# hku-mars/GS-SDF

Measured on NVIDIA H100. Metric: train_steps_per_s, higher is better.
Workload: dtype f32

## Files before the change

### gs-sdf_b200/csrc/sdf_grid.cuh

```cuda
#pragma once
#include <cuda_bf16.h>
#include <cuda_fp16.h>

#include "common.cuh"

namespace gssdf {

constexpr int kSdfThreads = 256;
constexpr int kMaxLevels = 16;
constexpr int kFeat = 32;

struct GridGeom {
    int L;
    uint32_t offset[kMaxLevels + 1];
    float scale[kMaxLevels];
    uint32_t res[kMaxLevels];
};

static inline float h_grid_scale(uint32_t level, float log2_pls, uint32_t base) { return exp2f(level * log2_pls) * base - 1.0f; }

static GridGeom make_grid(const gssdf_sdf_net &net) {
    GridGeom g;
    g.L = net.n_levels;
    uint32_t off = 0;
// ... 49 lines not shown
        p.pg[d] = (uint32_t)(int)t;
        p.pos[d] = v - t;
    }
    return p;
}

template <bool BRANCH_FREE = false>
__device__ __forceinline__ float2 encode_level(const __half2 *__restrict__ table, const GridGeom &g, int lvl, const float x[3]) {
    const __half2 *t = table + g.offset[lvl];
    const uint32_t hs = g.offset[lvl + 1] - g.offset[lvl];
    const LevelPos p = level_pos(x, g.scale[lvl]);
    __half2 vals[8];
    float w[8];
#pragma unroll
    for (int idx = 0; idx < 8; ++idx) {
        float wt = 1.f;
        uint32_t c[3];
#pragma unroll
        for (int d = 0; d < 3; ++d) {
            if ((idx & (1 << d)) == 0) { wt *= 1.f - p.pos[d]; c[d] = p.pg[d]; }
            else { wt *= p.pos[d]; c[d] = p.pg[d] + 1; }
        }
        w[idx] = wt;
        vals[idx] = __ldg(t + (BRANCH_FREE ? grid_index_sel : grid_index)(hs, g.res[lvl], c[0], c[1], c[2]));
    }
    __half2 r = __floats2half2_rn(0.f, 0.f);
#pragma unroll
    for (int idx = 0; idx < 8; ++idx) r = __hfma2(__float2half2_rn(w[idx]), vals[idx], r);
    return __half22float2(r);
}

struct Corners {
    uint32_t idx[8];
    float2 val[8];
};
__device__ __forceinline__ void load_corners(const __half2 *__restrict__ t, uint32_t hs, uint32_t res, const LevelPos &p, bool want_val, Corners &c) {
#pragma unroll
    for (int k = 0; k < 8; ++k)
        c.idx[k] = grid_index(hs, res, p.pg[0] + (k & 1), p.pg[1] + ((k >> 1) & 1), p.pg[2] + ((k >> 2) & 1));
    if (want_val) {
#pragma unroll
        for (int k = 0; k < 8; ++k) c.val[k] = __half22float2(__ldg(t + c.idx[k]));
    }
}
__device__ __forceinline__ int pair_left(int gd, int idx, const LevelPos &p, float &wt) {
    int cl = 0;
#pragma unroll
    for (int nd = 0; nd < 2; ++nd) {
        const int d = nd >= gd ? nd + 1 : nd;
        if ((idx & (1 << nd)) == 0) wt *= 1.f - p.pos[d];
        else { wt *= p.pos[d]; cl |= 1 << d; }
    }
    return cl;
}

__device__ __forceinline__ void encode_level_bwd(const __half2 *__restrict__ table, float *__restrict__ table_grad, const GridGeom &g,
                                                 int lvl, const float x[3], float g0, float g1, bool want_dx, float dx[3]) {
    const uint32_t hs = g.offset[lvl + 1] - g.offset[lvl];
    const LevelPos p = level_pos(x, g.scale[lvl]);
    const __half2 gh = __hmul2(__floats2half2_rn(g0, g1), __float2half2_rn(128.f));
    Corners c;
    load_corners(table + g.offset[lvl], hs, g.res[lvl], p, want_dx, c);
    if (table_grad) {
        float *tg = table_grad + 2 * (size_t)g.offset[lvl];
#pragma unroll
        for (int idx = 0; idx < 8; ++idx) {
            float wt = 1.f;
#pragma unroll
            for (int d = 0; d < 3; ++d) wt *= (idx & (1 << d)) == 0 ? 1.f - p.pos[d] : p.pos[d];
            const float2 v = __half22float2(__hmul2(__float2half2_rn(wt), gh));
            if (v.x != 0.f || v.y != 0.f)
                atomicAdd(reinterpret_cast<float2 *>(tg + 2 * (size_t)c.idx[idx]), make_float2(v.x * (1.f / 128.f), v.y * (1.f / 128.f)));
        }
    }
    if (want_dx) {
        const float2 ghf = __half22float2(gh);
#pragma unroll
        for (int gd = 0; gd < 3; ++gd) {
            float acc0 = 0.f, acc1 = 0.f;
#pragma unroll
            for (int idx = 0; idx < 4; ++idx) {
                float wt = g.scale[lvl];
                const int cl = pair_left(gd, idx, p, wt), cr = cl | (1 << gd);
                acc0 += wt * (c.val[cr].x - c.val[cl].x);
                acc1 += wt * (c.val[cr].y - c.val[cl].y);
            }
            dx[gd] = (ghf.x * acc0 + ghf.y * acc1) * (1.f / 128.f);
        }
    }
}

__device__ __forceinline__ void encode_level_bwd2(const __half2 *__restrict__ table, float *__restrict__ table_grad, const GridGeom &g,
                                                  int lvl, const float x[3], float dfeat0, float dfeat1, const float cc[3], float r[2]) {
    const uint32_t hs = g.offset[lvl + 1] - g.offset[lvl];
    const LevelPos p = level_pos(x, g.scale[lvl]);
    const __half2 gh = __hmul2(__floats2half2_rn(dfeat0, dfeat1), __float2half2_rn(128.f));
    Corners c;
    load_corners(table + g.offset[lvl], hs, g.res[lvl], p, true, c);
    float2 tacc[8];
#pragma unroll
    for (int k = 0; k < 8; ++k) tacc[k] = make_float2(0.f, 0.f);
    float r0 = 0.f, r1 = 0.f;
#pragma unroll
    for (int gd = 0; gd < 3; ++gd) {
        float acc0 = 0.f, acc1 = 0.f;
        const float grad_in = g.scale[lvl] * cc[gd];
#pragma unroll
        for (int idx = 0; idx < 4; ++idx) {
            float wd = g.scale[lvl], w = grad_in;
            const int cl = pair_left(gd, idx, p, wd);
            (void)pair_left(gd, idx, p, w);
            const int cr = cl | (1 << gd);
            acc0 += wd * (c.val[cr].x - c.val[cl].x);
            acc1 += wd * (c.val[cr].y - c.val[cl].y);
            if (table_grad) {
                const float2 vl = __half22float2(__hmul2(__float2half2_rn(-w), gh)), vr = __half22float2(__hmul2(__float2half2_rn(w), gh));
                tacc[cl].x += vl.x; tacc[cl].y += vl.y;
                tacc[cr].x += vr.x; tacc[cr].y += vr.y;
            }
        }
        r0 += acc0 * cc[gd];
        r1 += acc1 * cc[gd];
    }
    if (table_grad) {
        float *tg = table_grad + 2 * (size_t)g.offset[lvl];
#pragma unroll
        for (int k = 0; k < 8; ++k)
            if (tacc[k].x != 0.f || tacc[k].y != 0.f)
                atomicAdd(reinterpret_cast<float2 *>(tg + 2 * (size_t)c.idx[k]), make_float2(tacc[k].x * (1.f / 128.f), tacc[k].y * (1.f / 128.f)));
    }
    r[0] = __half2float(__float2half_rn(r0));
    r[1] = __half2float(__float2half_rn(r1));
}

__device__ __forceinline__ void load_x(const gssdf_sdf_net &net, const float *__restrict__ x, int64_t gi, int64_t n, float delta,
                                       float out[3]) {
    const int64_t i = gi % n;
    const int var = (int)(gi / n);
#pragma unroll
    for (int d = 0; d < 3; ++d) {
        float v = __ldg(x + 3 * i + d);
        if (var > 0 && (var - 1) / 2 == d) v += ((var - 1) & 1) ? -delta : delta;
        out[d] = net.inv_size != 0.f ? __fadd_rn(__fmul_rn(__fsub_rn(v, net.origin[d]), net.inv_size), 0.5f) : v;
    }
}


}
```

### gs-sdf_b200/csrc/sdf_tc.cu

```cuda
#include "sdf_grid.cuh"
#include "sdf_loss.cuh"

namespace gssdf {

constexpr int kFwdTcThreads = 512;
constexpr int kBwdTcThreads = 512;
constexpr int kLevels = 16;
static_assert(128 * kLevels == 4 * kBwdTcThreads, "encode batches assume 4 tasks per thread");
constexpr uint32_t kWImg = 24576;
constexpr uint32_t kGW = 3072;
constexpr uint32_t kGA = 2048;
constexpr uint32_t kGA0 = 1024;
constexpr uint32_t kGL = 1024;

__device__ __forceinline__ uint32_t off_act(int r, int k, int part) {
    return (uint32_t)((r >> 3) * kGA + part * 1024 + (k >> 3) * 128 + (r & 7) * 16 + (k & 7) * 2);
}
__device__ __forceinline__ uint32_t off_feat(int r, int k, int part) {
    return (uint32_t)((r >> 3) * kGA0 + part * 512 + (k >> 3) * 128 + (r & 7) * 16 + (k & 7) * 2);
}
__device__ __forceinline__ uint32_t off_lo(int r, int k) { return (uint32_t)((r >> 3) * kGL + (k >> 3) * 128 + (r & 7) * 16 + (k & 7) * 2); }
__device__ __host__ __forceinline__ uint32_t off_w(int o, int k, int part) {
    return (uint32_t)((o >> 3) * kGW + part * 1024 + (k >> 3) * 128 + (o & 7) * 16 + (k & 7) * 2);
}
// ... 295 lines not shown
                float act[32];
#pragma unroll
                for (int e = 0; e < 32; ++e) act[e] = fmaxf(d[e] + s_bias[l * 64 + 8 * (e >> 2) + fc + (e & 1)], 0.f);
                if (l < nh - 1) {
#pragma unroll
                    for (int e = 0; e < 32; e += 2) store2(sA, sL, fr + 8 * ((e >> 1) & 1), 8 * (e >> 2) + fc, act[e], act[e + 1]);
                } else {
                    float p0[2] = {0.f, 0.f}, p1[2] = {0.f, 0.f};
#pragma unroll
                    for (int e = 0; e < 32; ++e) {
                        const int i = (e >> 1) & 1, c = 8 * (e >> 2) + fc + (e & 1);
                        p0[i] = fmaf(act[e], s_wout[c], p0[i]);
                        p1[i] = fmaf(act[e], s_wout[HID + c], p1[i]);
                    }
#pragma unroll
                    for (int i = 0; i < 2; ++i) {
                        const float s0 = quad_sum(p0[i]), s1 = quad_sum(p1[i]);
                        const int p = fr + 8 * i;
                        bool live;
                        const int64_t e = eval_of(tile, p, live);
                        if ((lane & 3) == 0 && live) {
                            a.sdf[e] = s0 + s_wout[2 * HID];
                            if (a.y1) a.y1[e] = s1 + s_wout[2 * HID + 1];
                        }
                    }
                }
            }
            ++k;
        }
    }
    if (!ok) __trap();
}

constexpr size_t kBwdTcMain = 16 * kGA0 + 3 * 16 * kGA + 16 * kGA + 16 * kGL + kWImg;
constexpr size_t kBwdTcMisc = sizeof(float) * (4 * 64 + 132 + 384 + 4 * 128);
constexpr size_t kBwdTcMiscAnalytic = 128 * 16 * sizeof(uint16_t) + 128 * 3 * sizeof(float) + 64;
constexpr size_t bwd_tc_smem(bool analytic) { return kBwdTcMain + kBwdTcMisc + (analytic ? kBwdTcMiscAnalytic : 0); }
static_assert(bwd_tc_smem(true) + 1024 + 128 <= 196 * 1024, "the analytic variant must fit the 196 KiB shared-memory carve-out");

struct TcLossArgs {
    const float *gt_sdf, *weights, *visibilities;
    SdfLossCfg cfg;
    float *loss_out;
    int analytic;
    float align_weight;
    const float *sdf_variants;
    const uint8_t *valid_mask;
    const int32_t *n_gate;
};

template <bool FUSED, bool ANALYTIC>
__global__ void __launch_bounds__(kBwdTcThreads, 1)
sdf_bwd_tc_kernel(const gssdf_sdf_bwd_args a, const TcLossArgs lo, const GridGeom g, int64_t n_tiles) {
    constexpr int TM = 128, HID = 64, NT = kBwdTcThreads;
    extern __shared__ __align__(128) unsigned char s_tc[];
    unsigned char *sF = s_tc;
    unsigned char *sAct = sF + 16 * kGA0;
    unsigned char *sG = sAct + 3 * 16 * kGA;
    unsigned char *sL = sG + 16 * kGA;
    unsigned char *sW = sL + 16 * kGL;
    float *s_bias = reinterpret_cast<float *>(sW + kWImg);
    float *s_wout = s_bias + 4 * 64;
    float *s_dx = s_wout + 132;
    float *s_seed = s_dx;
    float *s_col = s_dx + 384;
    uint16_t *s_mask16 = reinterpret_cast<uint16_t *>(s_col + 4 * 128);
    float *s_gnum = s_col + 4 * 128 + 1024;
    int64_t *s_tbase = reinterpret_cast<int64_t *>(s_gnum + 384);
    __shared__ __align__(8) uint64_t s_wbar;

    const int tid = threadIdx.x, warp = tid >> 5, lane = tid & 31;
    const int q = warp & 3, cq = warp >> 2, row = 32 * q + lane, col0 = 16 * cq;
    const int wg = warp >> 2, fr = 16 * (warp & 3) + (lane >> 2), fc = 2 * (lane & 3);
    const int dr = 64 * (wg & 1) + fr, dc = 32 * (wg >> 1) + fc;
    const int nh = 1 + a.net.n_hidden;
    const int64_t n_eval = a.n * max(a.n_variants, 1);
    const int64_t n_live = a.n_live ? min((int64_t)*a.n_live, a.n) : a.n;
    const __half2 *table = reinterpret_cast<const __half2 *>(a.net.table_half);
    const unsigned char *wimg = reinterpret_cast<const unsigned char *>(a.net.mlp_packed);
    const int V = max(a.n_variants, 1), PT = FUSED ? TM / V : TM;
    float loss_acc = 0.f;
    constexpr bool analytic = ANALYTIC;
    static_assert(FUSED || !ANALYTIC, "the analytic eikonal path is part of the fused train kernel");
    float acc2_wo = 0.f;
    int n_coll = 0;

    if (tid == 0) {
        mbar_init(&s_wbar, 1);
        fence_mbar_init();
    }
    {
        const float *W = a.net.mlp;
        for (int l = 0; l < nh; ++l) {
            const int K = l == 0 ? kFeat : HID;
            if (tid < HID) s_bias[l * 64 + tid] = __ldg(W + (size_t)HID * K + tid);
            W += (size_t)HID * K + HID;
        }
        for (int e = tid; e < 2 * HID + 2; e += NT) s_wout[e] = __ldg(W + e);
    }
    __syncthreads();
    uint32_t ph_w = 0;
    bool ok = true, first_tile = true;
    float dbias[4] = {0.f, 0.f, 0.f, 0.f};
    float dwo0 = 0.f, dwo1 = 0.f, dbo = 0.f;
    float accW[32];
#pragma unroll
    for (int e = 0; e < 32; ++e) accW[e] = 0.f;
    float dD[16];

    auto sync_w = [&](bool wait) {
        fence_proxy_async();
        bool landed = true;
        if (wait) { landed = mbar_wait_bounded(&s_wbar, ph_w); ph_w ^= 1; }
        ok = __syncthreads_and(landed) && ok;
    };
    auto load_w = [&](int l) {
        mbar_arrive_expect_tx(&s_wbar, kWImg);
        bulk_g2s(sW, wimg + (size_t)l * kWImg, kWImg, &s_wbar);
    };
    auto finish = [&]() {
        wg_wait();
        acc_fence(dD);
        __syncthreads();
    };
    auto issue_gw = [&]() {
        const uint32_t gB = smem_u32(sG) + 8 * (wg & 1) * kGA, wB = smem_u32(sW) + 4 * (wg >> 1) * 128;
        wg_fence();
#pragma unroll
        for (int ks = 0; ks < HID / 16; ++ks) {
            const uint64_t gh = make_desc(gB + ks * 256, 128, kGA), gm = make_desc(gB + 1024 + ks * 256, 128, kGA);
            const uint64_t wh = make_desc(wB + ks * 2 * kGW, kGW, 128), wm = make_desc(wB + 1024 + ks * 2 * kGW, kGW, 128);
            wgmma_bf16<0, 1>(dD, gh, wh, ks > 0 ? 1u : 0u);
            wgmma_bf16<0, 1>(dD, gh, wm, 1);
            wgmma_bf16<0, 1>(dD, gm, wh, 1);
            wgmma_bf16<0, 1>(dD, gm, wm, 1);
        }
        wg_commit();
    };
    auto issue_dw = [&](int l) {
        if (wg != l) return;
        const uint32_t aB = smem_u32(l == 0 ? sF : sAct + (l - 1) * 16 * kGA), ga = l == 0 ? kGA0 : kGA, am = l == 0 ? 512u : 1024u;
        const uint32_t gB = smem_u32(sG);
        wg_fence();
#pragma unroll
        for (int ks = 0; ks < TM / 16; ++ks) {
            const uint64_t ah = make_desc(aB + ks * 2 * ga, ga, 128), amd = make_desc(aB + am + ks * 2 * ga, ga, 128);
            const uint64_t gh = make_desc(gB + ks * 2 * kGA, kGA, 128), gm = make_desc(gB + 1024 + ks * 2 * kGA, kGA, 128);
            wgmma_bf16<1, 1>(accW, ah, gh, 1);
            wgmma_bf16<1, 1>(accW, ah, gm, 1);
            wgmma_bf16<1, 1>(accW, amd, gh, 1);
            wgmma_bf16<1, 1>(accW, amd, gm, 1);
        }
        wg_commit();
    };


    auto second_order = [&]() {
        const int nc = n_coll;
        float *gf = reinterpret_cast<float *>(sL);
        float *s_cc = s_col;
        const float isz = a.net.inv_size != 0.f ? a.net.inv_size : 1.f;
        __syncthreads();
        for (int e = tid; e < (TM - nc) * 16; e += NT) s_mask16[nc * 16 + e] = 0;
        for (int e = tid; e < TM * 3; e += NT) s_dx[e] = 0.f;
        __syncthreads();
        auto seed_u = [&]() {
            const uint32_t bits = s_mask16[(row * 4 + nh - 1) * 4 + cq];
            float u[16];
#pragma unroll
            for (int j = 0; j < 16; ++j) u[j] = ((bits >> j) & 1u) ? s_wout[col0 + j] : 0.f;
            store8(sG, nullptr, row, col0, u);
            store8(sG, nullptr, row, col0 + 8, u + 8);
        };
        auto mask_bit = [&](int slot, int l, int e) -> bool {
            const int j = e >> 2;
            return (s_mask16[(slot * 4 + l - 1) * 4 + 2 * (wg >> 1) + (j >> 1)] >> (8 * (j & 1) + fc + (e & 1))) & 1u;
        };
        auto mask_store = [&](int l, unsigned char *dst) {
#pragma unroll
            for (int e = 0; e < 16; e += 2) {
                const int r = dr + 8 * ((e >> 1) & 1);
                store2(dst, nullptr, r, dc + 8 * (e >> 2), mask_bit(r, l, e) ? dD[e] : 0.f, mask_bit(r, l, e + 1) ? dD[e + 1] : 0.f);
            }
        };
        auto store_gf = [&]() {
            if (wg >> 1) return;
#pragma unroll
            for (int e = 0; e < 16; ++e) gf[(dr + 8 * ((e >> 1) & 1)) * 33 + dc + 8 * (e >> 2) + (e & 1)] = dD[e];
        };
        seed_u();
        if (tid == 0) { fence_proxy_async(); load_w(nh - 1); }
        for (int l = nh - 1; l >= 0 && ok; --l) {
            sync_w(true);
            if (!ok) return;
            issue_gw();
            finish();
            if (tid == 0 && l > 0) load_w(l - 1);
            if (l > 0) mask_store(l, sG);
            else store_gf();
        }
        __syncthreads();
        {
            static_assert(NT % TM == 0, "thread -> point mapping of the analytic pass");
            const int c = tid % TM;
            if (c < nc) {
                float x[3], acc[3] = {0.f, 0.f, 0.f};
                load_x(a.net, a.x, s_tbase[c / PT] + c % PT, a.n, a.delta, x);
#pragma unroll 1
                for (int lvl = tid / TM; lvl < kLevels; lvl += NT / TM) {
                    float dx[3] = {0.f, 0.f, 0.f};
                    encode_level_bwd(table, nullptr, g, lvl, x, gf[c * 33 + 2 * lvl], gf[c * 33 + 2 * lvl + 1], true, dx);
                    acc[0] += dx[0]; acc[1] += dx[1]; acc[2] += dx[2];
                }
                atomicAdd(&s_dx[c * 3 + 0], acc[0]);
                atomicAdd(&s_dx[c * 3 + 1], acc[1]);
                atomicAdd(&s_dx[c * 3 + 2], acc[2]);
            }
        }
        __syncthreads();
        if (tid < TM) {
            float cc[3] = {0.f, 0.f, 0.f};
            const SdfGate gate = tid < nc ? sdf_gate(lo.n_gate, lo.valid_mask, lo.visibilities, lo.cfg.visible_thr, s_tbase[tid / PT] + tid % PT)
                                          : SdfGate{false, true, 1.f};
            if (tid < nc && (!gate.gated || gate.gate)) {
                const float gx = s_dx[tid * 3] * isz, gy = s_dx[tid * 3 + 1] * isz, gz = s_dx[tid * 3 + 2] * isz;
                const float nl = gate.gated ? gate.ng : (float)n_live;
                const float nrm = sqrtf(gx * gx + gy * gy + gz * gz);
                const float we = lo.cfg.eikonal_weight / nl;
                loss_acc += we * (nrm - 1.f) * (nrm - 1.f);
                const float ke = nrm > 0.f ? 2.f * (nrm - 1.f) / nrm * we : 0.f;
                cc[0] = ke * gx; cc[1] = ke * gy; cc[2] = ke * gz;
                if (lo.align_weight > 0.f && (V == 7 || lo.sdf_variants)) {
                    const float wa = lo.align_weight / (3.f * nl);
                    const float *gn = s_gnum + tid * 3;
                    const float d0 = gx - gn[0], d1 = gy - gn[1], d2 = gz - gn[2];
                    loss_acc += wa * (fabsf(d0) + fabsf(d1) + fabsf(d2));
                    cc[0] += d0 > 0.f ? wa : (d0 < 0.f ? -wa : 0.f);
                    cc[1] += d1 > 0.f ? wa : (d1 < 0.f ? -wa : 0.f);
                    cc[2] += d2 > 0.f ? wa : (d2 < 0.f ? -wa : 0.f);
                }
            }
            s_cc[tid * 3] = cc[0] * isz; s_cc[tid * 3 + 1] = cc[1] * isz; s_cc[tid * 3 + 2] = cc[2] * isz;
        }
        __syncthreads();
#pragma unroll 1
        for (int task = tid; task < TM * kLevels; task += NT) {
            const int c = task % TM, lvl = task / TM;
            float r[2] = {0.f, 0.f};
            if (c < nc) {
                float x[3];
                load_x(a.net, a.x, s_tbase[c / PT] + c % PT, a.n, a.delta, x);
                encode_level_bwd2(table, a.table_grad, g, lvl, x, gf[c * 33 + 2 * lvl], gf[c * 33 + 2 * lvl + 1], s_cc + c * 3, r);
            }
            __nv_bfloat16 h0, m0, h1, m1;
            split2(r[0], h0, m0);
            split2(r[1], h1, m1);
            *reinterpret_cast<__nv_bfloat162 *>(sF + off_feat(c, 2 * lvl, 0)) = __halves2bfloat162(h0, h1);
            *reinterpret_cast<__nv_bfloat162 *>(sF + off_feat(c, 2 * lvl, 1)) = __halves2bfloat162(m0, m1);
        }
        if (!a.mlp_grad) { __syncthreads(); return; }
        __syncthreads();
        if (tid == 0) { fence_proxy_async(); load_w(0); }
        for (int l = 0; l < nh; ++l) {
            sync_w(true);
            if (!ok) return;
            issue_forward_layer<false>(dD, l, smem_u32(l == 0 ? sF + 8 * (wg & 1) * kGA0 : sAct + (l - 1) * 16 * kGA + 8 * (wg & 1) * kGA),
                                       0u, smem_u32(sW) + 4 * (wg >> 1) * kGW);
            finish();
            if (tid == 0 && (l + 1 < nh || nh > 1)) load_w(l + 1 < nh ? l + 1 : nh - 1);
            if (l < nh - 1) {
                mask_store(l + 1, sAct + l * 16 * kGA);
            } else {
#pragma unroll
                for (int e = 0; e < 16; e += 4) {
#pragma unroll
                    for (int c = 0; c < 2; ++c) {
                        float s = (mask_bit(dr, nh, e + c) ? dD[e + c] : 0.f) + (mask_bit(dr + 8, nh, e + 2 + c) ? dD[e + 2 + c] : 0.f);
                        s += __shfl_xor_sync(0xffffffffu, s, 4);
                        s += __shfl_xor_sync(0xffffffffu, s, 8);
                        s += __shfl_xor_sync(0xffffffffu, s, 16);
                        if (lane < 4) s_col[(4 * (wg & 1) + (warp & 3)) * 64 + dc + 2 * e + c] = s;
                    }
                }
            }
        }
        __syncthreads();
        if (q == 0 && lane < 16) {
            const int c = col0 + lane;
#pragma unroll
            for (int rg = 0; rg < 8; ++rg) acc2_wo += s_col[rg * 64 + c];
        }
        seed_u();
        for (int l = nh - 1; l >= 0 && ok; --l) {
            sync_w(l > 0);
            if (!ok) return;
            issue_dw(l);
            if (l > 0) issue_gw();
            finish();
            if (tid == 0 && l > 1) load_w(l - 1);
            if (l > 0) mask_store(l, sG);
        }
        __syncthreads();
    };

    for (int64_t tile = blockIdx.x; tile < n_tiles && ok; tile += gridDim.x) {
        const int64_t base = FUSED ? tile * PT : tile * TM;
        const int tm = (int)min((int64_t)TM, n_eval - base);
        if (FUSED ? base >= n_live : (base % a.n >= n_live && base % a.n + TM <= a.n)) continue;
        auto row_gi = [&](int p) -> int64_t {
            if (!FUSED) return min(base + p, n_eval - 1);
            const int j = p / V, v = p - j * V;
            return (int64_t)v * a.n + min(base + j, a.n - 1);
        };
        auto row_live = [&](int p) -> bool {
            if (!FUSED) return p < tm && (base + p) % a.n < n_live;
            const int j = p / V;
            return j < PT && base + j < n_live;
        };
        auto row_is_base = [&](int p) -> bool { return FUSED ? (p % V) == 0 : base + p < a.n; };
#define LIVE_TC(p_) row_live(p_)
        __syncthreads();
        if (tid == 0) {
            fence_proxy_async();
            load_w(0);
        }
        {
            float2 f[4];
#pragma unroll
            for (int i = 0; i < 4; ++i) {
                const int task = i * NT + tid, p = task % TM, lvl = task / TM;
                float x[3];
                load_x(a.net, a.x, row_gi(p), a.n, a.delta, x);
                f[i] = encode_level(table, g, lvl, x);
            }
#pragma unroll
            for (int i = 0; i < 4; ++i) {
                const int task = i * NT + tid, p = task % TM, lvl = task / TM;
                if (!LIVE_TC(p)) f[i] = make_float2(0.f, 0.f);
                __nv_bfloat16 h0, m0, h1, m1;
                split2(f[i].x, h0, m0);
                split2(f[i].y, h1, m1);
                *reinterpret_cast<__nv_bfloat162 *>(sF + off_feat(p, 2 * lvl, 0)) = __halves2bfloat162(h0, h1);
                *reinterpret_cast<__nv_bfloat162 *>(sF + off_feat(p, 2 * lvl, 1)) = __halves2bfloat162(m0, m1);
            }
        }
        if (!FUSED && tid < TM) {
            const bool lv = LIVE_TC(tid);
            s_seed[2 * tid] = lv ? __ldg(a.v_sdf + base + tid) : 0.f;
            s_seed[2 * tid + 1] = (lv && a.v_y1) ? __ldg(a.v_y1 + base + tid) : 0.f;
        }
        for (int l = 0; l < nh; ++l) {
            sync_w(true);
            if (!ok) break;
            issue_forward_layer(dD, l, smem_u32(l == 0 ? sF + 8 * (wg & 1) * kGA0 : sAct + (l - 1) * 16 * kGA + 8 * (wg & 1) * kGA),
                                smem_u32(sL + 8 * (wg & 1) * kGL), smem_u32(sW) + 4 * (wg >> 1) * kGW);
            finish();
            if (tid == 0 && l + 1 < nh) load_w(l + 1);
            float act[16];
#pragma unroll
            for (int e = 0; e < 16; ++e) act[e] = fmaxf(dD[e] + s_bias[l * 64 + dc + 8 * (e >> 2) + (e & 1)], 0.f);
            unsigned char *dst = (l < nh - 1) ? sAct + l * 16 * kGA : sG;
#pragma unroll
            for (int e = 0; e < 16; e += 2) store2(dst, l < nh - 1 ? sL : nullptr, dr + 8 * ((e >> 1) & 1), dc + 8 * (e >> 2), act[e], act[e + 1]);
            if (analytic) {
#pragma unroll
                for (int i = 0; i < 2; ++i) {
                    uint32_t bits[2] = {0u, 0u};
#pragma unroll
                    for (int j = 0; j < 4; ++j)
#pragma unroll
                        for (int c = 0; c < 2; ++c) bits[j >> 1] |= (act[4 * j + 2 * i + c] > 0.f ? 1u : 0u) << (8 * (j & 1) + fc + c);
#pragma unroll
                    for (int h = 0; h < 2; ++h) {
                        bits[h] |= __shfl_xor_sync(0xffffffffu, bits[h], 1);
                        bits[h] |= __shfl_xor_sync(0xffffffffu, bits[h], 2);
                    }
                    const int r = dr + 8 * i, jb = r / V;
                    if ((lane & 3) == 0 && r - jb * V == 0 && jb < PT && base + jb < n_live) {
                        s_mask16[((n_coll + jb) * 4 + l) * 4 + 2 * (wg >> 1)] = (uint16_t)bits[0];
                        s_mask16[((n_coll + jb) * 4 + l) * 4 + 2 * (wg >> 1) + 1] = (uint16_t)bits[1];
                    }
                }
            }
            if (FUSED && l == nh - 1) {
                float p0[2] = {0.f, 0.f}, p1[2] = {0.f, 0.f};
#pragma unroll
                for (int e = 0; e < 16; ++e) {
                    const int i = (e >> 1) & 1, c = dc + 8 * (e >> 2) + (e & 1);
                    p0[i] = fmaf(act[e], s_wout[c], p0[i]);
                    p1[i] = fmaf(act[e], s_wout[HID + c], p1[i]);
                }
                float *s_part = reinterpret_cast<float *>(sL);
#pragma unroll
                for (int i = 0; i < 2; ++i) {
                    const float s0 = quad_sum(p0[i]), s1 = quad_sum(p1[i]);
                    if ((lane & 3) == 0) {
                        s_part[((wg >> 1) * TM + dr + 8 * i) * 2] = s0;
                        s_part[((wg >> 1) * TM + dr + 8 * i) * 2 + 1] = s1;
                    }
                }
            }
        }
        if (!ok) break;
        __syncthreads();
        if (FUSED) {
            float *s_part = reinterpret_cast<float *>(sL), *s_out = s_part + 2 * TM * 2;
            if (tid < TM) {
                s_out[2 * tid] = s_part[tid * 2] + s_part[(TM + tid) * 2] + s_wout[2 * HID];
                s_out[2 * tid + 1] = s_part[tid * 2 + 1] + s_part[(TM + tid) * 2 + 1] + s_wout[2 * HID + 1];
                s_seed[2 * tid] = 0.f;
                s_seed[2 * tid + 1] = 0.f;
            }
            __syncthreads();
            if (tid < PT && base + tid < n_live) {
                const int64_t i = base + tid;
                float sv[7], v_s[7], v_y;
                for (int v = 0; v < V; ++v) sv[v] = s_out[2 * (tid * V + v)];
                SdfLossCfg cfg1 = lo.cfg;
                if (analytic) {
                    cfg1.eikonal_weight = 0.f;
                    if (tid == 0) s_tbase[n_coll / PT] = base;
                    if (V == 1 && lo.sdf_variants) {
                        for (int v = 1; v < 7; ++v) sv[v] = __ldg(lo.sdf_variants + (int64_t)v * a.n + i);
                    }
                    if (V == 7 || lo.sdf_variants) {
                        const float inv2d = 0.5f / lo.cfg.delta;
                        s_gnum[(n_coll + tid) * 3 + 0] = (sv[1] - sv[2]) * inv2d;
                        s_gnum[(n_coll + tid) * 3 + 1] = (sv[3] - sv[4]) * inv2d;
                        s_gnum[(n_coll + tid) * 3 + 2] = (sv[5] - sv[6]) * inv2d;
                    }
                }
                loss_acc += sdf_point_loss(cfg1, (float)n_live, V, sv, s_out[2 * tid * V + 1], lo.gt_sdf != nullptr,
                                           lo.gt_sdf ? __ldg(lo.gt_sdf + i) : 0.f, lo.weights != nullptr, lo.weights ? __ldg(lo.weights + i) : 0.f,
                                           lo.visibilities != nullptr, lo.visibilities ? __ldg(lo.visibilities + i) : 0.f, v_s, v_y,
                                           sdf_gate(lo.n_gate, lo.valid_mask, lo.visibilities, lo.cfg.visible_thr, i));
                for (int v = 0; v < V; ++v) s_seed[2 * (tid * V + v)] = v_s[v];
                s_seed[2 * tid * V + 1] = v_y;
            }
            __syncthreads();
        }
        {
            float an[16], gl[16];
            load8_sum(sG, row, col0, an);
            load8_sum(sG, row, col0 + 8, an + 8);
            const float v0 = s_seed[2 * row], v1 = s_seed[2 * row + 1];
#pragma unroll
            for (int j = 0; j < 16; ++j) gl[j] = an[j] > 0.f ? v0 * s_wout[col0 + j] + v1 * s_wout[HID + col0 + j] : 0.f;
            store8(sG, nullptr, row, col0, gl);
            store8(sG, nullptr, row, col0 + 8, gl + 8);
            if (a.mlp_grad) {
                float c0[16], c1[16];
#pragma unroll
                for (int j = 0; j < 16; ++j) { c0[j] = v0 * an[j]; c1[j] = v1 * an[j]; }
                const float s0 = colsum16(c0, lane), s1 = colsum16(c1, lane);
                if (lane < 16) {
                    s_col[q * 128 + col0 + lane] = s0;
                    s_col[q * 128 + 64 + col0 + lane] = s1;
                }
                if (cq == 0) {
                    const float b0 = warp_sum(v0), b1 = warp_sum(v1);
                    if (lane == 0) { s_dx[256 + 2 * q] = b0; s_dx[256 + 2 * q + 1] = b1; }
                }
            }
        }
        __syncthreads();
        if (a.mlp_grad) {
            if (tid < 2 * HID) {
                const float s = s_col[tid] + s_col[128 + tid] + s_col[256 + tid] + s_col[384 + tid];
                if (tid < HID) dwo0 += s; else dwo1 += s;
            } else if (tid < 2 * HID + 2) {
                const int o = tid - 2 * HID;
                dbo += s_dx[256 + o] + s_dx[258 + o] + s_dx[260 + o] + s_dx[262 + o];
            }
        }
        for (int l = nh - 1; l >= 0; --l) {
            sync_w(l < nh - 1);
            if (!ok) break;
            if (a.mlp_grad) issue_dw(l);
            issue_gw();
            if (a.mlp_grad) {
                float c[16];
                load8_sum(sG, row, col0, c);
                load8_sum(sG, row, col0 + 8, c + 8);
                const float s = colsum16(c, lane);
                if (lane < 16) s_col[q * 128 + col0 + lane] = s;
            }
            finish();
            if (tid == 0 && l > 0) load_w(l - 1);
            if (l > 0) {
#pragma unroll
                for (int e = 0; e < 16; e += 2) {
                    const int r = dr + 8 * ((e >> 1) & 1), c = dc + 8 * (e >> 2);
                    const float2 m = load2_hi(sAct + (l - 1) * 16 * kGA, r, c);
                    store2(sG, nullptr, r, c, m.x > 0.f ? dD[e] : 0.f, m.y > 0.f ? dD[e + 1] : 0.f);
                }
            } else if ((wg >> 1) == 0) {
                float *gf = reinterpret_cast<float *>(sL);
#pragma unroll
                for (int e = 0; e < 16; ++e) gf[(dr + 8 * ((e >> 1) & 1)) * 33 + dc + 8 * (e >> 2) + (e & 1)] = dD[e];
            }
            __syncthreads();
            if (a.mlp_grad && q == 0 && lane < 16) {
                const int c = col0 + lane;
                dbias[l] += s_col[c] + s_col[128 + c] + s_col[256 + c] + s_col[384 + c];
            }
        }
        if (!ok) break;
        for (int e = tid; e < TM * 3; e += NT) s_dx[e] = 0.f;
        __syncthreads();
        {
            const float *gf = reinterpret_cast<const float *>(sL);
            for (int task = tid; task < TM * g.L; task += NT) {
                const int p = task % TM, lvl = task / TM;
                if (LIVE_TC(p)) {
                    float x[3], dx[3] = {0.f, 0.f, 0.f};
                    load_x(a.net, a.x, row_gi(p), a.n, a.delta, x);
                    const bool want_dx = a.v_x != nullptr && row_is_base(p);
                    encode_level_bwd(table, a.table_grad, g, lvl, x, gf[p * 33 + 2 * lvl], gf[p * 33 + 2 * lvl + 1], want_dx, dx);
                    if (want_dx) {
                        atomicAdd(&s_dx[p * 3 + 0], dx[0]);
                        atomicAdd(&s_dx[p * 3 + 1], dx[1]);
                        atomicAdd(&s_dx[p * 3 + 2], dx[2]);
                    }
                }
            }
        }
        __syncthreads();
        if (a.v_x) {
            const float sc = a.net.inv_size != 0.f ? a.net.inv_size : 1.f;
            if (FUSED) {
                for (int e = tid; e < PT * 3; e += NT) {
                    const int j = e / 3, d = e - 3 * j;
                    if (base + j < n_live) a.v_x[(base + j) * 3 + d] = s_dx[(j * V) * 3 + d] * sc;
                }
            } else {
                for (int e = tid; e < tm * 3; e += NT)
                    if (base + e / 3 < n_live) a.v_x[base * 3 + e] = s_dx[e] * sc;
            }
        }
        first_tile = false;
        if (ANALYTIC) {
            n_coll += (int)min((int64_t)PT, n_live - base);
            if (n_coll + PT > TM) {
                second_order();
                n_coll = 0;
                if (!ok) break;
            }
        }

#undef LIVE_TC
    }
    if (ANALYTIC && ok && n_coll > 0) second_order();
    __syncthreads();
    if (ok && a.mlp_grad && !first_tile) {
        float *G = a.mlp_grad;
        for (int l = 0; l < nh; ++l) {
            const int K = l == 0 ? kFeat : HID;
            if (wg == l) {
#pragma unroll
                for (int e = 0; e < 32; ++e) {
                    const int k = fr + 8 * ((e >> 1) & 1), o = 8 * (e >> 2) + fc + (e & 1);
                    if (k < K) atomicAdd(G + (size_t)o * K + k, accW[e]);
                }
            }
            if (q == 0 && lane < 16) atomicAdd(G + (size_t)HID * K + col0 + lane, dbias[l]);
            G += (size_t)HID * K + HID;
        }
        if (ANALYTIC && q == 0 && lane < 16) atomicAdd(G + col0 + lane, acc2_wo);
        if (tid < HID) atomicAdd(G + tid, dwo0);
        else if (tid < 2 * HID) atomicAdd(G + tid, dwo1);
        else if (tid < 2 * HID + 2) atomicAdd(G + tid, dbo);
    }
    if (FUSED && lo.loss_out) {
        loss_acc = warp_sum(loss_acc);
        if (lane == 0 && loss_acc != 0.f) atomicAdd(lo.loss_out, loss_acc);
    }
    if (!ok) __trap();
}

}

using namespace gssdf;

extern "C" int64_t gssdf_sdf_mlp_packed_bytes(const gssdf_sdf_net *net) {
    if (!net || net->hidden_dim != 64 || net->n_hidden < 0 || net->n_hidden > 3) return -1;
    return (int64_t)(1 + net->n_hidden) * kWImg;
}

extern "C" int gssdf_sdf_mlp_pack(const gssdf_sdf_net *net, void *packed, gssdf_stream_t stream) {
    GSSDF_REQUIRE(net && packed, GSSDF_EINVAL, "sdf_mlp_pack: null argument");
    GSSDF_REQUIRE(net->hidden_dim == 64 && net->n_levels * net->n_features_per_level == kFeat, GSSDF_EUNSUPPORTED,
                  "sdf_mlp_pack: the tensor-core decoder needs hidden_dim 64 and 32 encoded features");
    GSSDF_REQUIRE(net->n_hidden >= 0 && net->n_hidden <= 3, GSSDF_EUNSUPPORTED, "sdf_mlp_pack: n_hidden %d not in [0,3]", net->n_hidden);
    GSSDF_REQUIRE(net->mlp, GSSDF_EINVAL, "sdf_mlp_pack: net.mlp is null");
    GSSDF_REQUIRE(((uintptr_t)packed & 15) == 0, GSSDF_EINVAL, "sdf_mlp_pack: packed must be 16-byte aligned");
    mlp_pack_kernel<<<1 + net->n_hidden, 256, 0, (cudaStream_t)stream>>>(net->mlp, reinterpret_cast<unsigned char *>(packed), 1 + net->n_hidden);
    GSSDF_LAUNCH_OK("mlp_pack_kernel");
    return GSSDF_OK;
}

static int check_tc(const char *who, const gssdf_sdf_net &net) {
    GSSDF_REQUIRE(net.hidden_dim == 64, GSSDF_EUNSUPPORTED, "%s: the tensor-core decoder needs hidden_dim 64", who);
    GSSDF_REQUIRE(net.n_hidden <= 3, GSSDF_EUNSUPPORTED, "%s: the tensor-core decoder supports n_hidden <= 3 (one weight-gradient accumulator per warpgroup)", who);
    GSSDF_REQUIRE(net.mlp_packed && ((uintptr_t)net.mlp_packed & 15) == 0, GSSDF_EINVAL,
                  "%s: mlp_mode 1 needs net.mlp_packed (gssdf_sdf_mlp_pack), 16-byte aligned", who);
    return GSSDF_OK;
}

extern "C" int gssdf_sdf_fwd_tc_launch(const gssdf_sdf_fwd_args *a, const gssdf::GridGeom *g, gssdf_stream_t stream) {
    int rc = check_tc("sdf_fwd", a->net);
    if (rc) return rc;
    static bool attr_set = false;
    if (!attr_set) {
        GSSDF_CUDA_OK(cudaFuncSetAttribute(sdf_fwd_tc_kernel, cudaFuncAttributeMaxDynamicSharedMemorySize, (int)kFwdTcSmem));
        attr_set = true;
    }
    const int nv = a->n_variants > 1 ? a->n_variants : 1, pt = 128 / (nv == 7 && a->skip_base_variant ? 6 : nv);
    const int64_t n_tiles = (a->n + pt - 1) / pt;
    int dev = 0, sms = 132;
    cudaGetDevice(&dev);
    cudaDeviceGetAttribute(&sms, cudaDevAttrMultiProcessorCount, dev);
    const int grid = (int)std::min<int64_t>(n_tiles, (int64_t)sms);
    sdf_fwd_tc_kernel<<<grid, kFwdTcThreads, kFwdTcSmem, (cudaStream_t)stream>>>(*a, *g, n_tiles);
    GSSDF_LAUNCH_OK("sdf_fwd_tc_kernel");
    return GSSDF_OK;
}

extern "C" int gssdf_sdf_bwd_tc_launch(const gssdf_sdf_bwd_args *a, const gssdf::GridGeom *g, gssdf_stream_t stream) {
    int rc = check_tc("sdf_bwd", a->net);
    if (rc) return rc;
    GSSDF_CUDA_OK(cudaFuncSetAttribute(sdf_bwd_tc_kernel<false, false>, cudaFuncAttributeMaxDynamicSharedMemorySize, (int)bwd_tc_smem(false)));
    const int64_t n_tiles = (a->n * (a->n_variants > 1 ? a->n_variants : 1) + 127) / 128;
    int dev = 0, sms = 132;
    cudaGetDevice(&dev);
    cudaDeviceGetAttribute(&sms, cudaDevAttrMultiProcessorCount, dev);
    const int grid = (int)std::min<int64_t>(n_tiles, (int64_t)sms);
    sdf_bwd_tc_kernel<false, false><<<grid, kBwdTcThreads, bwd_tc_smem(false), (cudaStream_t)stream>>>(*a, TcLossArgs{}, *g, n_tiles);
    GSSDF_LAUNCH_OK("sdf_bwd_tc_kernel");
    return GSSDF_OK;
}

extern "C" int gssdf_sdf_train(const gssdf_sdf_train_args *t, gssdf_stream_t stream) {
    GSSDF_REQUIRE(t != nullptr, GSSDF_EINVAL, "sdf_train: null args");
    GSSDF_REQUIRE(t->net.mlp_mode == 1, GSSDF_EUNSUPPORTED, "sdf_train: the fused forward+loss+backward kernel exists for mlp_mode 1 only "
                  "(use gssdf_sdf_fwd + gssdf_sdf_loss + gssdf_sdf_bwd otherwise)");
    GSSDF_REQUIRE(t->net.n_levels == 16 && t->net.n_features_per_level == 2, GSSDF_EUNSUPPORTED, "sdf_train: 16 levels x 2 features only");
    int rc = check_tc("sdf_train", t->net);
    if (rc) return rc;
    GSSDF_REQUIRE(t->n >= 0, GSSDF_EINVAL, "sdf_train: negative n");
    if (t->n == 0) return GSSDF_OK;
    GSSDF_REQUIRE(t->x && t->net.table_half && t->net.mlp, GSSDF_EINVAL, "sdf_train: x, table_half, mlp must be non-null");
    GSSDF_REQUIRE(t->n_variants == 1 || t->n_variants == 7, GSSDF_EINVAL, "sdf_train: n_variants must be 1 or 7");
    GSSDF_REQUIRE(t->n_variants == 1 || t->delta > 0.f, GSSDF_EINVAL, "sdf_train: delta must be positive");
    GSSDF_REQUIRE(((uintptr_t)t->table_grad & 7) == 0, GSSDF_EINVAL, "sdf_train: table_grad must be 8-byte aligned");
    gssdf_sdf_bwd_args a{};
    a.net = t->net; a.n = t->n; a.x = t->x; a.n_variants = t->n_variants; a.delta = t->delta; a.n_live = t->n_live;
    a.table_grad = t->table_grad; a.mlp_grad = t->mlp_grad; a.v_x = t->v_x;
    TcLossArgs lo{t->gt_sdf, t->weights, t->visibilities,
                  SdfLossCfg{t->bce_isigma, t->bce_weight, t->eikonal_weight, t->gs_sdf_weight, t->delta, t->visible_thr}, t->loss_out,
                  t->eikonal_mode, t->align_weight, t->n_variants == 1 ? t->sdf_variants : nullptr, t->valid_mask, t->n_gate};
    GSSDF_REQUIRE(t->eikonal_mode == 0 || t->eikonal_mode == 1, GSSDF_EINVAL, "sdf_train: eikonal_mode must be 0 or 1");
    GSSDF_REQUIRE(!(t->eikonal_mode == 1 && t->align_weight > 0.f) || t->n_variants == 7 || t->sdf_variants, GSSDF_EINVAL,
                  "sdf_train: the align loss needs the numerical gradient: n_variants 7 or sdf_variants");
    GSSDF_REQUIRE(!t->sdf_variants || t->delta > 0.f, GSSDF_EINVAL, "sdf_train: sdf_variants needs the delta they were evaluated with");
    GSSDF_REQUIRE(t->eikonal_mode == 1 || t->align_weight == 0.f, GSSDF_EINVAL, "sdf_train: align_weight needs eikonal_mode 1");
    const GridGeom g = make_grid(t->net);
    GSSDF_CUDA_OK(cudaFuncSetAttribute(sdf_bwd_tc_kernel<true, false>, cudaFuncAttributeMaxDynamicSharedMemorySize, (int)bwd_tc_smem(false)));
    GSSDF_CUDA_OK(cudaFuncSetAttribute(sdf_bwd_tc_kernel<true, true>, cudaFuncAttributeMaxDynamicSharedMemorySize, (int)bwd_tc_smem(true)));
    const int pt = 128 / t->n_variants;
    const int64_t n_tiles = (t->n + pt - 1) / pt;
    int dev = 0, sms = 132;
    cudaGetDevice(&dev);
    cudaDeviceGetAttribute(&sms, cudaDevAttrMultiProcessorCount, dev);
// ... 9 lines not shown
```

Before: 209.7.

## Fold first-order grid backward into analytic second-order passes and batch corner gathers

When the analytic eikonal path runs with a single variant, the first-order hash-grid backward pass (table-gradient scatter and input-gradient) is no longer a separate loop. It is folded into the existing second-order passes, so corner indices and values are gathered once per level and the per-level atomics are combined into one set. Feature gradients are stored as half2 in a level-major layout, corner values stay in half2, two levels are gathered together to raise memory-level parallelism, and one __syncthreads is dropped. Optional clock64 phase instrumentation is added behind a compile flag. Costs include more registers and a small precision change from storing feature gradients as half.

```diff
diff --git a/gs-sdf_b200/csrc/sdf_grid.cuh b/gs-sdf_b200/csrc/sdf_grid.cuh
--- a/gs-sdf_b200/csrc/sdf_grid.cuh
+++ b/gs-sdf_b200/csrc/sdf_grid.cuh
@@ -105,15 +105,16 @@
 
 struct Corners {
     uint32_t idx[8];
-    float2 val[8];
+    __half2 val[8];
 };
+template <bool BRANCH_FREE = false>
 __device__ __forceinline__ void load_corners(const __half2 *__restrict__ t, uint32_t hs, uint32_t res, const LevelPos &p, bool want_val, Corners &c) {
 #pragma unroll
     for (int k = 0; k < 8; ++k)
-        c.idx[k] = grid_index(hs, res, p.pg[0] + (k & 1), p.pg[1] + ((k >> 1) & 1), p.pg[2] + ((k >> 2) & 1));
+        c.idx[k] = (BRANCH_FREE ? grid_index_sel : grid_index)(hs, res, p.pg[0] + (k & 1), p.pg[1] + ((k >> 1) & 1), p.pg[2] + ((k >> 2) & 1));
     if (want_val) {
 #pragma unroll
-        for (int k = 0; k < 8; ++k) c.val[k] = __half22float2(__ldg(t + c.idx[k]));
+        for (int k = 0; k < 8; ++k) c.val[k] = __ldg(t + c.idx[k]);
     }
 }
 __device__ __forceinline__ int pair_left(int gd, int idx, const LevelPos &p, float &wt) {
@@ -125,6 +126,22 @@
         else { wt *= p.pos[d]; cl |= 1 << d; }
     }
     return cl;
+}
+__device__ __forceinline__ void level_dydx(float scale, const LevelPos &p, const __half2 val[8], float d0[3], float d1[3]) {
+#pragma unroll
+    for (int gd = 0; gd < 3; ++gd) {
+        float acc0 = 0.f, acc1 = 0.f;
+#pragma unroll
+        for (int idx = 0; idx < 4; ++idx) {
+            float wt = scale;
+            const int cl = pair_left(gd, idx, p, wt), cr = cl | (1 << gd);
+            const float2 vl = __half22float2(val[cl]), vr = __half22float2(val[cr]);
+            acc0 += wt * (vr.x - vl.x);
+            acc1 += wt * (vr.y - vl.y);
+        }
+        d0[gd] = acc0;
+        d1[gd] = acc1;
+    }
 }
 
 __device__ __forceinline__ void encode_level_bwd(const __half2 *__restrict__ table, float *__restrict__ table_grad, const GridGeom &g,
@@ -148,19 +165,53 @@
     }
     if (want_dx) {
         const float2 ghf = __half22float2(gh);
-#pragma unroll
-        for (int gd = 0; gd < 3; ++gd) {
-            float acc0 = 0.f, acc1 = 0.f;
+        float d0[3], d1[3];
+        level_dydx(g.scale[lvl], p, c.val, d0, d1);
+#pragma unroll
+        for (int gd = 0; gd < 3; ++gd) dx[gd] = (ghf.x * d0[gd] + ghf.y * d1[gd]) * (1.f / 128.f);
+    }
+}
+
+__device__ __forceinline__ void level_bwd2(float *__restrict__ tg, float scale, const LevelPos &p, const Corners &c, __half2 gh, bool first,
+                                           __half2 gh1, const float cc[3], float r[2]) {
+    float2 tacc[8];
+#pragma unroll
+    for (int k = 0; k < 8; ++k) {
+        tacc[k] = make_float2(0.f, 0.f);
+        if (first) {
+            float wt = 1.f;
+#pragma unroll
+            for (int d = 0; d < 3; ++d) wt *= (k & (1 << d)) == 0 ? 1.f - p.pos[d] : p.pos[d];
+            tacc[k] = __half22float2(__hmul2(__float2half2_rn(wt), gh1));
+        }
+    }
+    float d0[3], d1[3];
+    level_dydx(scale, p, c.val, d0, d1);
+    float r0 = 0.f, r1 = 0.f;
+#pragma unroll
+    for (int gd = 0; gd < 3; ++gd) {
+        const float grad_in = scale * cc[gd];
+        if (tg) {
 #pragma unroll
             for (int idx = 0; idx < 4; ++idx) {
-                float wt = g.scale[lvl];
-                const int cl = pair_left(gd, idx, p, wt), cr = cl | (1 << gd);
-                acc0 += wt * (c.val[cr].x - c.val[cl].x);
-                acc1 += wt * (c.val[cr].y - c.val[cl].y);
+                float w = grad_in;
+                const int cl = pair_left(gd, idx, p, w), cr = cl | (1 << gd);
+                const float2 vl = __half22float2(__hmul2(__float2half2_rn(-w), gh)), vr = __half22float2(__hmul2(__float2half2_rn(w), gh));
+                tacc[cl].x += vl.x; tacc[cl].y += vl.y;
+                tacc[cr].x += vr.x; tacc[cr].y += vr.y;
             }
-            dx[gd] = (ghf.x * acc0 + ghf.y * acc1) * (1.f / 128.f);
-        }
-    }
+        }
+        r0 += d0[gd] * cc[gd];
+        r1 += d1[gd] * cc[gd];
+    }
+    if (tg) {
+#pragma unroll
+        for (int k = 0; k < 8; ++k)
+            if (tacc[k].x != 0.f || tacc[k].y != 0.f)
+                atomicAdd(reinterpret_cast<float2 *>(tg + 2 * (size_t)c.idx[k]), make_float2(tacc[k].x * (1.f / 128.f), tacc[k].y * (1.f / 128.f)));
+    }
+    r[0] = __half2float(__float2half_rn(r0));
+    r[1] = __half2float(__float2half_rn(r1));
 }
 
 __device__ __forceinline__ void encode_level_bwd2(const __half2 *__restrict__ table, float *__restrict__ table_grad, const GridGeom &g,
@@ -170,40 +221,7 @@
     const __half2 gh = __hmul2(__floats2half2_rn(dfeat0, dfeat1), __float2half2_rn(128.f));
     Corners c;
     load_corners(table + g.offset[lvl], hs, g.res[lvl], p, true, c);
-    float2 tacc[8];
-#pragma unroll
-    for (int k = 0; k < 8; ++k) tacc[k] = make_float2(0.f, 0.f);
-    float r0 = 0.f, r1 = 0.f;
-#pragma unroll
-    for (int gd = 0; gd < 3; ++gd) {
-        float acc0 = 0.f, acc1 = 0.f;
-        const float grad_in = g.scale[lvl] * cc[gd];
-#pragma unroll
-        for (int idx = 0; idx < 4; ++idx) {
-            float wd = g.scale[lvl], w = grad_in;
-            const int cl = pair_left(gd, idx, p, wd);
-            (void)pair_left(gd, idx, p, w);
-            const int cr = cl | (1 << gd);
-            acc0 += wd * (c.val[cr].x - c.val[cl].x);
-            acc1 += wd * (c.val[cr].y - c.val[cl].y);
-            if (table_grad) {
-                const float2 vl = __half22float2(__hmul2(__float2half2_rn(-w), gh)), vr = __half22float2(__hmul2(__float2half2_rn(w), gh));
-                tacc[cl].x += vl.x; tacc[cl].y += vl.y;
-                tacc[cr].x += vr.x; tacc[cr].y += vr.y;
-            }
-        }
-        r0 += acc0 * cc[gd];
-        r1 += acc1 * cc[gd];
-    }
-    if (table_grad) {
-        float *tg = table_grad + 2 * (size_t)g.offset[lvl];
-#pragma unroll
-        for (int k = 0; k < 8; ++k)
-            if (tacc[k].x != 0.f || tacc[k].y != 0.f)
-                atomicAdd(reinterpret_cast<float2 *>(tg + 2 * (size_t)c.idx[k]), make_float2(tacc[k].x * (1.f / 128.f), tacc[k].y * (1.f / 128.f)));
-    }
-    r[0] = __half2float(__float2half_rn(r0));
-    r[1] = __half2float(__float2half_rn(r1));
+    level_bwd2(table_grad ? table_grad + 2 * (size_t)g.offset[lvl] : nullptr, g.scale[lvl], p, c, gh, false, gh, cc, r);
 }
 
 __device__ __forceinline__ void load_x(const gssdf_sdf_net &net, const float *__restrict__ x, int64_t gi, int64_t n, float delta,
diff --git a/gs-sdf_b200/csrc/sdf_tc.cu b/gs-sdf_b200/csrc/sdf_tc.cu
--- a/gs-sdf_b200/csrc/sdf_tc.cu
+++ b/gs-sdf_b200/csrc/sdf_tc.cu
@@ -351,6 +351,25 @@
     if (!ok) __trap();
 }
 
+constexpr int kPassBatch = 2;
+static_assert((128 * kLevels / kBwdTcThreads) % kPassBatch == 0, "pass batches cover a thread's levels");
+
+enum SdfTrainPhase { kPhEncode, kPhForward, kPhLoss, kPhHidden, kPhStep5, kPhUChain, kPhPassA, kPhEikonal, kPhPassB, kPhQChain, kPhUChain2,
+                     kPhRest, kNumSdfTrainPhases };
+#ifdef GSSDF_SDF_TRAIN_PHASES
+__device__ unsigned long long g_sdf_train_phase_cycles[kNumSdfTrainPhases];
+#define SDF_PHASE(k_)                                                                        \
+    do {                                                                                     \
+        if (tid == 0) {                                                                      \
+            const long long t_ = clock64();                                                  \
+            atomicAdd(&g_sdf_train_phase_cycles[k_], (unsigned long long)(t_ - ph_t0));      \
+            ph_t0 = t_;                                                                      \
+        }                                                                                    \
+    } while (0)
+#else
+#define SDF_PHASE(k_) do {} while (0)
+#endif
+
 constexpr size_t kBwdTcMain = 16 * kGA0 + 3 * 16 * kGA + 16 * kGA + 16 * kGL + kWImg;
 constexpr size_t kBwdTcMisc = sizeof(float) * (4 * 64 + 132 + 384 + 4 * 128);
 constexpr size_t kBwdTcMiscAnalytic = 128 * 16 * sizeof(uint16_t) + 128 * 3 * sizeof(float) + 64;
@@ -377,6 +396,7 @@
     unsigned char *sAct = sF + 16 * kGA0;
     unsigned char *sG = sAct + 3 * 16 * kGA;
     unsigned char *sL = sG + 16 * kGA;
+    __half2 *gf1 = reinterpret_cast<__half2 *>(sL), *gfu = gf1 + kLevels * TM;
     unsigned char *sW = sL + 16 * kGL;
     float *s_bias = reinterpret_cast<float *>(sW + kWImg);
     float *s_wout = s_bias + 4 * 64;
@@ -403,6 +423,10 @@
     static_assert(FUSED || !ANALYTIC, "the analytic eikonal path is part of the fused train kernel");
     float acc2_wo = 0.f;
     int n_coll = 0;
+    const bool fold = ANALYTIC && V == 1;
+#ifdef GSSDF_SDF_TRAIN_PHASES
+    long long ph_t0 = clock64();
+#endif
 
     if (tid == 0) {
         mbar_init(&s_wbar, 1);
@@ -442,6 +466,11 @@
         acc_fence(dD);
         __syncthreads();
     };
+    auto store_dfeat = [&](__half2 *dst) {
+        if (wg >> 1) return;
+#pragma unroll
+        for (int e = 0; e < 16; e += 2) dst[((dc + 8 * (e >> 2)) >> 1) * TM + dr + 8 * ((e >> 1) & 1)] = __floats2half2_rn(dD[e], dD[e + 1]);
+    };
     auto issue_gw = [&]() {
         const uint32_t gB = smem_u32(sG) + 8 * (wg & 1) * kGA, wB = smem_u32(sW) + 4 * (wg >> 1) * 128;
         wg_fence();
@@ -476,12 +505,13 @@
 
     auto second_order = [&]() {
         const int nc = n_coll;
-        float *gf = reinterpret_cast<float *>(sL);
         float *s_cc = s_col;
+        float *s_dx1 = s_col;
+        const bool first_dx = fold && a.v_x != nullptr;
         const float isz = a.net.inv_size != 0.f ? a.net.inv_size : 1.f;
         __syncthreads();
         for (int e = tid; e < (TM - nc) * 16; e += NT) s_mask16[nc * 16 + e] = 0;
-        for (int e = tid; e < TM * 3; e += NT) s_dx[e] = 0.f;
+        for (int e = tid; e < TM * 3; e += NT) s_dx[e] = s_dx1[e] = 0.f;
         __syncthreads();
         auto seed_u = [&]() {
             const uint32_t bits = s_mask16[(row * 4 + nh - 1) * 4 + cq];
@@ -501,11 +531,6 @@
                 const int r = dr + 8 * ((e >> 1) & 1);
                 store2(dst, nullptr, r, dc + 8 * (e >> 2), mask_bit(r, l, e) ? dD[e] : 0.f, mask_bit(r, l, e + 1) ? dD[e + 1] : 0.f);
             }
-        };
-        auto store_gf = [&]() {
-            if (wg >> 1) return;
-#pragma unroll
-            for (int e = 0; e < 16; ++e) gf[(dr + 8 * ((e >> 1) & 1)) * 33 + dc + 8 * (e >> 2) + (e & 1)] = dD[e];
         };
         seed_u();
         if (tid == 0) { fence_proxy_async(); load_w(nh - 1); }
@@ -516,28 +541,56 @@
             finish();
             if (tid == 0 && l > 0) load_w(l - 1);
             if (l > 0) mask_store(l, sG);
-            else store_gf();
+            else store_dfeat(gfu);
         }
         __syncthreads();
-        {
-            static_assert(NT % TM == 0, "thread -> point mapping of the analytic pass");
-            const int c = tid % TM;
-            if (c < nc) {
-                float x[3], acc[3] = {0.f, 0.f, 0.f};
-                load_x(a.net, a.x, s_tbase[c / PT] + c % PT, a.n, a.delta, x);
+        SDF_PHASE(kPhUChain);
+        static_assert(NT % TM == 0, "thread -> point mapping of the analytic passes");
+        constexpr int kLvlStep = NT / TM;
+        const int c = tid % TM;
+        float x[3];
+        if (c < nc) load_x(a.net, a.x, s_tbase[c / PT] + c % PT, a.n, a.delta, x);
+        auto gather = [&](int lvl, LevelPos &p, Corners &cr) {
+            p = level_pos(x, g.scale[lvl]);
+            load_corners<true>(table + g.offset[lvl], g.offset[lvl + 1] - g.offset[lvl], g.res[lvl], p, true, cr);
+        };
+        const __half2 h128 = __float2half2_rn(128.f);
+        if (c < nc) {
+            float acc[3] = {0.f, 0.f, 0.f}, acc1[3] = {0.f, 0.f, 0.f};
 #pragma unroll 1
-                for (int lvl = tid / TM; lvl < kLevels; lvl += NT / TM) {
-                    float dx[3] = {0.f, 0.f, 0.f};
-                    encode_level_bwd(table, nullptr, g, lvl, x, gf[c * 33 + 2 * lvl], gf[c * 33 + 2 * lvl + 1], true, dx);
-                    acc[0] += dx[0]; acc[1] += dx[1]; acc[2] += dx[2];
-                }
-                atomicAdd(&s_dx[c * 3 + 0], acc[0]);
-                atomicAdd(&s_dx[c * 3 + 1], acc[1]);
-                atomicAdd(&s_dx[c * 3 + 2], acc[2]);
+            for (int l0 = tid / TM; l0 < kLevels; l0 += kPassBatch * kLvlStep) {
+                LevelPos p[kPassBatch];
+                Corners cr[kPassBatch];
+#pragma unroll
+                for (int i = 0; i < kPassBatch; ++i) gather(l0 + i * kLvlStep, p[i], cr[i]);
+#pragma unroll
+                for (int i = 0; i < kPassBatch; ++i) {
+                    const int lvl = l0 + i * kLvlStep;
+                    float d0[3], d1[3];
+                    level_dydx(g.scale[lvl], p[i], cr[i].val, d0, d1);
+                    const float2 gu = __half22float2(__hmul2(gfu[lvl * TM + c], h128));
+#pragma unroll
+                    for (int gd = 0; gd < 3; ++gd) acc[gd] += (gu.x * d0[gd] + gu.y * d1[gd]) * (1.f / 128.f);
+                    if (first_dx) {
+                        const float2 g1 = __half22float2(__hmul2(gf1[lvl * TM + c], h128));
+#pragma unroll
+                        for (int gd = 0; gd < 3; ++gd) acc1[gd] += (g1.x * d0[gd] + g1.y * d1[gd]) * (1.f / 128.f);
+                    }
+                }
+            }
+#pragma unroll
+            for (int gd = 0; gd < 3; ++gd) {
+                atomicAdd(&s_dx[c * 3 + gd], acc[gd]);
+                if (first_dx) atomicAdd(&s_dx1[c * 3 + gd], acc1[gd]);
             }
         }
         __syncthreads();
+        SDF_PHASE(kPhPassA);
         if (tid < TM) {
+            if (first_dx && tid < nc) {
+#pragma unroll
+                for (int d = 0; d < 3; ++d) a.v_x[(s_tbase[tid / PT] + tid % PT) * 3 + d] = s_dx1[tid * 3 + d] * isz;
+            }
             float cc[3] = {0.f, 0.f, 0.f};
             const SdfGate gate = tid < nc ? sdf_gate(lo.n_gate, lo.valid_mask, lo.visibilities, lo.cfg.visible_thr, s_tbase[tid / PT] + tid % PT)
                                           : SdfGate{false, true, 1.f};
@@ -562,14 +615,16 @@
             s_cc[tid * 3] = cc[0] * isz; s_cc[tid * 3 + 1] = cc[1] * isz; s_cc[tid * 3 + 2] = cc[2] * isz;
         }
         __syncthreads();
+        SDF_PHASE(kPhEikonal);
 #pragma unroll 1
-        for (int task = tid; task < TM * kLevels; task += NT) {
-            const int c = task % TM, lvl = task / TM;
+        for (int lvl = tid / TM; lvl < kLevels; lvl += kLvlStep) {
             float r[2] = {0.f, 0.f};
             if (c < nc) {
-                float x[3];
-                load_x(a.net, a.x, s_tbase[c / PT] + c % PT, a.n, a.delta, x);
-                encode_level_bwd2(table, a.table_grad, g, lvl, x, gf[c * 33 + 2 * lvl], gf[c * 33 + 2 * lvl + 1], s_cc + c * 3, r);
+                LevelPos p;
+                Corners cr;
+                gather(lvl, p, cr);
+                const __half2 gh = __hmul2(gfu[lvl * TM + c], h128), gh1 = fold ? __hmul2(gf1[lvl * TM + c], h128) : gh;
+                level_bwd2(a.table_grad ? a.table_grad + 2 * (size_t)g.offset[lvl] : nullptr, g.scale[lvl], p, cr, gh, fold, gh1, s_cc + c * 3, r);
             }
             __nv_bfloat16 h0, m0, h1, m1;
             split2(r[0], h0, m0);
@@ -577,8 +632,8 @@
             *reinterpret_cast<__nv_bfloat162 *>(sF + off_feat(c, 2 * lvl, 0)) = __halves2bfloat162(h0, h1);
             *reinterpret_cast<__nv_bfloat162 *>(sF + off_feat(c, 2 * lvl, 1)) = __halves2bfloat162(m0, m1);
         }
+        SDF_PHASE(kPhPassB);
         if (!a.mlp_grad) { __syncthreads(); return; }
-        __syncthreads();
         if (tid == 0) { fence_proxy_async(); load_w(0); }
         for (int l = 0; l < nh; ++l) {
             sync_w(true);
@@ -604,6 +659,7 @@
             }
         }
         __syncthreads();
+        SDF_PHASE(kPhQChain);
         if (q == 0 && lane < 16) {
             const int c = col0 + lane;
 #pragma unroll
@@ -620,6 +676,7 @@
             if (l > 0) mask_store(l, sG);
         }
         __syncthreads();
+        SDF_PHASE(kPhUChain2);
     };
 
     for (int64_t tile = blockIdx.x; tile < n_tiles && ok; tile += gridDim.x) {
@@ -668,6 +725,7 @@
             s_seed[2 * tid] = lv ? __ldg(a.v_sdf + base + tid) : 0.f;
             s_seed[2 * tid + 1] = (lv && a.v_y1) ? __ldg(a.v_y1 + base + tid) : 0.f;
         }
+        SDF_PHASE(kPhEncode);
         for (int l = 0; l < nh; ++l) {
             sync_w(true);
             if (!ok) break;
@@ -722,6 +780,7 @@
         }
         if (!ok) break;
         __syncthreads();
+        SDF_PHASE(kPhForward);
         if (FUSED) {
             float *s_part = reinterpret_cast<float *>(sL), *s_out = s_part + 2 * TM * 2;
             if (tid < TM) {
@@ -758,6 +817,7 @@
             }
             __syncthreads();
         }
+        SDF_PHASE(kPhLoss);
         {
             float an[16], gl[16];
             load8_sum(sG, row, col0, an);
@@ -813,10 +873,8 @@
                     const float2 m = load2_hi(sAct + (l - 1) * 16 * kGA, r, c);
                     store2(sG, nullptr, r, c, m.x > 0.f ? dD[e] : 0.f, m.y > 0.f ? dD[e + 1] : 0.f);
                 }
-            } else if ((wg >> 1) == 0) {
-                float *gf = reinterpret_cast<float *>(sL);
-#pragma unroll
-                for (int e = 0; e < 16; ++e) gf[(dr + 8 * ((e >> 1) & 1)) * 33 + dc + 8 * (e >> 2) + (e & 1)] = dD[e];
+            } else {
+                store_dfeat(gf1);
             }
             __syncthreads();
             if (a.mlp_grad && q == 0 && lane < 16) {
@@ -825,17 +883,18 @@
             }
         }
         if (!ok) break;
-        for (int e = tid; e < TM * 3; e += NT) s_dx[e] = 0.f;
-        __syncthreads();
-        {
-            const float *gf = reinterpret_cast<const float *>(sL);
+        SDF_PHASE(kPhHidden);
+        if (!fold) {
+            for (int e = tid; e < TM * 3; e += NT) s_dx[e] = 0.f;
+            __syncthreads();
             for (int task = tid; task < TM * g.L; task += NT) {
                 const int p = task % TM, lvl = task / TM;
                 if (LIVE_TC(p)) {
                     float x[3], dx[3] = {0.f, 0.f, 0.f};
                     load_x(a.net, a.x, row_gi(p), a.n, a.delta, x);
                     const bool want_dx = a.v_x != nullptr && row_is_base(p);
-                    encode_level_bwd(table, a.table_grad, g, lvl, x, gf[p * 33 + 2 * lvl], gf[p * 33 + 2 * lvl + 1], want_dx, dx);
+                    const float2 gv = __half22float2(gf1[lvl * TM + p]);
+                    encode_level_bwd(table, a.table_grad, g, lvl, x, gv.x, gv.y, want_dx, dx);
                     if (want_dx) {
                         atomicAdd(&s_dx[p * 3 + 0], dx[0]);
                         atomicAdd(&s_dx[p * 3 + 1], dx[1]);
@@ -843,9 +902,9 @@
                     }
                 }
             }
-        }
-        __syncthreads();
-        if (a.v_x) {
+            __syncthreads();
+        }
+        if (a.v_x && !fold) {
             const float sc = a.net.inv_size != 0.f ? a.net.inv_size : 1.f;
             if (FUSED) {
                 for (int e = tid; e < PT * 3; e += NT) {
@@ -857,6 +916,7 @@
                     if (base + e / 3 < n_live) a.v_x[base * 3 + e] = s_dx[e] * sc;
             }
         }
+        SDF_PHASE(kPhStep5);
         first_tile = false;
         if (ANALYTIC) {
             n_coll += (int)min((int64_t)PT, n_live - base);
@@ -894,8 +954,10 @@
         loss_acc = warp_sum(loss_acc);
         if (lane == 0 && loss_acc != 0.f) atomicAdd(lo.loss_out, loss_acc);
     }
+    SDF_PHASE(kPhRest);
     if (!ok) __trap();
 }
+#undef SDF_PHASE
 
 }
 
@@ -958,6 +1020,15 @@
     GSSDF_LAUNCH_OK("sdf_bwd_tc_kernel");
     return GSSDF_OK;
 }
+
+#ifdef GSSDF_SDF_TRAIN_PHASES
+extern "C" int gssdf_sdf_train_phases(unsigned long long *out) {
+    GSSDF_CUDA_OK(cudaMemcpyFromSymbol(out, g_sdf_train_phase_cycles, sizeof(g_sdf_train_phase_cycles)));
+    const unsigned long long zero[kNumSdfTrainPhases] = {};
+    GSSDF_CUDA_OK(cudaMemcpyToSymbol(g_sdf_train_phase_cycles, zero, sizeof(zero)));
+    return kNumSdfTrainPhases;
+}
+#endif
 
 extern "C" int gssdf_sdf_train(const gssdf_sdf_train_args *t, gssdf_stream_t stream) {
     GSSDF_REQUIRE(t != nullptr, GSSDF_EINVAL, "sdf_train: null args");
```

After: 213.7, median of 6. +1.9%, better.
